# nicoloalbergoni/DeepLabV3Plus-Augmented-SuperResolution

Measured on AMD Instinct MI355X. Metric: augmented-copies/sec (fwd+realign+SR-iter) @512x512, higher is better.
Workload: dtype f32 (pointwise GEMMs: operands split into f16 hi+lo, hi*hi+hi*lo+lo*hi on f16 MFMA, f32 accumulate)

## Files before the change

### deeplabv3plus-augmented-superresolution_amd/csrc/dwconv.hip

```cpp
#include "asr_common.h"

typedef float f32x4 __attribute__((ext_vector_type(4)));

namespace {

struct DwArgs {
    const float* x;
    const float* w;
    const float* bias;
    float* y;
    int batch, h_in, w_in, c, h_out, w_out;
    int stride, rate, pad_top, pad_left;
    int pre_relu, post_relu;
    int ldx, ldy;
};

__device__ __forceinline__ f32x4 relu4(f32x4 v) {
    v.x = fmaxf(v.x, 0.f); v.y = fmaxf(v.y, 0.f); v.z = fmaxf(v.z, 0.f); v.w = fmaxf(v.w, 0.f);
    return v;
}
__device__ __forceinline__ f32x4 post_act4(f32x4 v, int mode) {
    if (mode) v = relu4(v);
    if (mode == 2) { v.x = fminf(v.x, 6.f); v.y = fminf(v.y, 6.f); v.z = fminf(v.z, 6.f); v.w = fminf(v.w, 6.f); }
    return v;
}

constexpr int SCOLS = 16;

template <int R, int S, int SROWS>
__global__ __launch_bounds__(256) void dw_stream_kernel(DwArgs p, int tiles_x) {
    constexpr int WIN = 2 * R + 1;
    const int tid = threadIdx.x;
    const int c4 = tid & 15, col = tid >> 4;
    const int tx = blockIdx.x % tiles_x, cbk = blockIdx.x / tiles_x;
    const int ch = (cbk * 16 + c4) * 4;
    const int ox = tx * SCOLS + col;
    const int oy0 = blockIdx.y * SROWS;
    const int b = blockIdx.z;
    if (ch >= p.c || ox >= p.w_out) return;
    const float* xin = p.x + (long long)b * p.h_in * p.w_in * p.ldx + ch;
    float* yout = p.y + (long long)b * p.h_out * p.w_out * p.ldy + ch;
    f32x4 wk[9];
#pragma unroll
    for (int t = 0; t < 9; ++t) wk[t] = *reinterpret_cast<const f32x4*>(p.w + (long long)t * p.c + ch);
    const f32x4 bv = *reinterpret_cast<const f32x4*>(p.bias + ch);
    const int ixl = ox * S - p.pad_left, ixc = ixl + R, ixr = ixl + 2 * R;
    const bool vl = ixl >= 0 && ixl < p.w_in, vc = ixc >= 0 && ixc < p.w_in, vr = ixr >= 0 && ixr < p.w_in;
    const f32x4 zero = {0.f, 0.f, 0.f, 0.f};

    auto load_row = [&](int iy, f32x4& l, f32x4& c, f32x4& r) {
        l = zero; c = zero; r = zero;
        if (iy >= 0 && iy < p.h_in) {
            const float* row = xin + (long long)iy * p.w_in * p.ldx;
            if (vl) l = *reinterpret_cast<const f32x4*>(row + (long long)ixl * p.ldx);
            if (vc) c = *reinterpret_cast<const f32x4*>(row + (long long)ixc * p.ldx);
            if (vr) r = *reinterpret_cast<const f32x4*>(row + (long long)ixr * p.ldx);
        }
    };
    auto act = [&](const f32x4& v) { return p.pre_relu ? relu4(v) : v; };

    f32x4 win[WIN][3], nxt[S][3];
    const int base0 = oy0 * S - p.pad_top;
#pragma unroll
    for (int k = 0; k < WIN - S; ++k) {
        load_row(base0 + k, win[S + k][0], win[S + k][1], win[S + k][2]);
        win[S + k][0] = act(win[S + k][0]); win[S + k][1] = act(win[S + k][1]); win[S + k][2] = act(win[S + k][2]);
    }
#pragma unroll
    for (int j = 0; j < S; ++j) load_row(base0 + WIN - S + j, nxt[j][0], nxt[j][1], nxt[j][2]);
    const int rows = min(SROWS, p.h_out - oy0);
    for (int r = 0; r < rows; ++r) {
#pragma unroll
        for (int k = 0; k < WIN - S; ++k) { win[k][0] = win[k + S][0]; win[k][1] = win[k + S][1]; win[k][2] = win[k + S][2]; }
#pragma unroll
        for (int j = 0; j < S; ++j) { win[WIN - S + j][0] = act(nxt[j][0]); win[WIN - S + j][1] = act(nxt[j][1]); win[WIN - S + j][2] = act(nxt[j][2]); }
        if (r + 1 < rows) {
#pragma unroll
            for (int j = 0; j < S; ++j) load_row(base0 + r * S + WIN + j, nxt[j][0], nxt[j][1], nxt[j][2]);
        }
        f32x4 acc = bv;
#pragma unroll
        for (int ky = 0; ky < 3; ++ky)
#pragma unroll
            for (int kx = 0; kx < 3; ++kx) acc += win[ky * R][kx] * wk[ky * 3 + kx];
        acc = post_act4(acc, p.post_relu);
        *reinterpret_cast<f32x4*>(yout + ((long long)(oy0 + r) * p.w_out + ox) * p.ldy) = acc;
    }
}

typedef _Float16 f16x4 __attribute__((ext_vector_type(4)));

#ifndef ASR_DIAG_DW
#define ASR_DIAG_DW 0
#endif
#ifndef ASR_DW_PACKED_SPLIT
#define ASR_DW_PACKED_SPLIT 1
#endif
typedef unsigned int dw_u32x2 __attribute__((ext_vector_type(2)));
__device__ __forceinline__ void dw_split4(const f32x4& acc, dw_u32x2& h2, dw_u32x2& l2) {
#if ASR_DW_PACKED_SPLIT
    unsigned int h01, h23, l01, l23;
    asr_split4_f16_saturating_mode(acc[0], acc[1], acc[2], acc[3], h01, h23, l01, l23);
    h2 = dw_u32x2{h01, h23};
    l2 = dw_u32x2{l01, l23};
#else
    f16x4 hi, lo;
#pragma unroll
    for (int e = 0; e < 4; ++e) {
        _Float16 h, l;
        asr_split_f16(acc[e], h, l);
        hi[e] = h;
        lo[e] = l;
    }
    h2 = __builtin_bit_cast(dw_u32x2, hi);
    l2 = __builtin_bit_cast(dw_u32x2, lo);
#endif
}

#ifndef ASR_DW_NT
#define ASR_DW_NT 1
#endif
constexpr bool kNtStores = ASR_DW_NT != 0;
#ifndef ASR_DW_SMALL_MAX
#define ASR_DW_SMALL_MAX 64
#endif
template <int R, int S, int SROWS, int PF, bool SPLIT, int ACT>
__global__ __launch_bounds__(256) ASR_PK_F32 void dw_stream_full_kernel(DwArgs p, int tiles_x) {
    constexpr int WIN = 2 * R + 1;
    static_assert(SROWS % PF == 0, "strip length must be a multiple of the prefetch depth");
#if ASR_DW_PACKED_SPLIT
    if (SPLIT) asr_enable_f16_saturation();
#endif
    const int tid = threadIdx.x;
    const int c4 = tid & 15, col = tid >> 4;
    const int tx = blockIdx.x % tiles_x, cbk = blockIdx.x / tiles_x;
    const int ch = (cbk * 16 + c4) * 4;
    const int ox = tx * SCOLS + col;
    const int oy0 = blockIdx.y * SROWS;
    const int b = blockIdx.z;
    _Float16* ysplit = nullptr;
    long long split_row_stride = 0;
    if (SPLIT) {
        ysplit = reinterpret_cast<_Float16*>(p.y) + (((long long)b * p.h_out * p.w_out + ox) * p.ldy + (ch >> 5)) * 64 + (ch & 31);
        split_row_stride = (long long)p.w_out * p.ldy * 64;
        if (ox < p.w_out && ch >= p.c && ch < p.ldy * 32) {
            const f16x4 z = {(_Float16)0.f, (_Float16)0.f, (_Float16)0.f, (_Float16)0.f};
            for (int r = 0; r < SROWS; ++r) {
                _Float16* o = ysplit + (long long)(oy0 + r) * split_row_stride;
                *reinterpret_cast<f16x4*>(o) = z;
                *reinterpret_cast<f16x4*>(o + 32) = z;
            }
        }
    }
    if (ch >= p.c || ox >= p.w_out) return;
    const float* xin = p.x + (long long)b * p.h_in * p.w_in * p.ldx + ch;
    float* yout = p.y + ((long long)b * p.h_out * p.w_out + ox) * p.ldy + ch;
    const int ixl = ox * S - p.pad_left, ixc = ixl + R, ixr = ixl + 2 * R;
    const bool vl = ixl >= 0 && ixl < p.w_in, vc = ixc >= 0 && ixc < p.w_in, vr = ixr >= 0 && ixr < p.w_in;
    const f32x4 zero = {0.f, 0.f, 0.f, 0.f};
    f32x4 wk[9];
#pragma unroll
    for (int t = 0; t < 9; ++t) {
        const bool col_ok = (t % 3 == 0) ? vl : ((t % 3 == 1) ? vc : vr);
        const f32x4 wv = *reinterpret_cast<const f32x4*>(p.w + (long long)t * p.c + ch);
        wk[t] = col_ok ? wv : zero;
    }
    const f32x4 bv = *reinterpret_cast<const f32x4*>(p.bias + ch);
    const long long ofl = (long long)min(max(ixl, 0), p.w_in - 1) * p.ldx, ofc = (long long)min(max(ixc, 0), p.w_in - 1) * p.ldx,
                    ofr = (long long)min(max(ixr, 0), p.w_in - 1) * p.ldx;
    const long long row_stride = (long long)p.w_in * p.ldx;
    const bool pre = ACT == 0 ? p.pre_relu != 0 : ACT == 1;

    auto issue = [&](int iy, f32x4 (&d)[3]) {
        const float* row = xin + (long long)min(max(iy, 0), p.h_in - 1) * row_stride;
#if ASR_DIAG_DW & 4
        d[1] = *reinterpret_cast<const f32x4*>(row + ofc);
        d[0] = d[1]; d[2] = d[1];
#else
        d[0] = *reinterpret_cast<const f32x4*>(row + ofl);
        d[1] = *reinterpret_cast<const f32x4*>(row + ofc);
        d[2] = *reinterpret_cast<const f32x4*>(row + ofr);
#endif
    };
    auto enter = [&](int iy, const f32x4 (&d)[3], f32x4 (&w)[3]) {
        const int vy = __builtin_amdgcn_readfirstlane((int)(iy >= 0 && iy < p.h_in));
#pragma unroll
        for (int k = 0; k < 3; ++k) w[k] = (ACT == 1) ? relu4(d[k]) : ((ACT == 2) ? d[k] : (pre ? relu4(d[k]) : d[k]));
        if (!vy) {
            asm volatile("" ::: "memory");
            w[0] = zero; w[1] = zero; w[2] = zero;
        }
    };

    f32x4 win[WIN][3], q[PF][S][3];
    const int base0 = oy0 * S - p.pad_top;
#pragma unroll
    for (int k = 0; k < WIN - S; ++k) {
        f32x4 d[3];
        issue(base0 + k, d);
        enter(base0 + k, d, win[S + k]);
    }
#pragma unroll
    for (int j = 0; j < PF; ++j)
#pragma unroll
        for (int t = 0; t < S; ++t) issue(base0 + WIN - S + j * S + t, q[j][t]);
#pragma unroll
    for (int r0 = 0; r0 < SROWS; r0 += PF) {
#pragma unroll
        for (int j = 0; j < PF; ++j) {
            const int r = r0 + j;
#pragma unroll
            for (int k = 0; k < WIN - S; ++k) { win[k][0] = win[k + S][0]; win[k][1] = win[k + S][1]; win[k][2] = win[k + S][2]; }
#pragma unroll
            for (int t = 0; t < S; ++t) enter(base0 + r * S + WIN - S + t, q[j][t], win[WIN - S + t]);
#pragma unroll
            for (int t = 0; t < S; ++t) issue(base0 + (r + PF) * S + WIN - S + t, q[j][t]);
            f32x4 acc = bv;
#if ASR_DIAG_DW & 1
            acc += win[R][1] * wk[4] + win[0][0] + win[2 * R][2];
#else
#pragma unroll
            for (int ky = 0; ky < 3; ++ky)
#pragma unroll
                for (int kx = 0; kx < 3; ++kx) acc += win[ky * R][kx] * wk[ky * 3 + kx];
#endif
            if (ACT == 2) acc = relu4(acc);
            else if (ACT == 0) acc = post_act4(acc, p.post_relu);
#if ASR_DIAG_DW & 2
            if (SPLIT) {
                _Float16* o = ysplit + (long long)(oy0 + r) * split_row_stride + ((c4 & 1) ? 32 - 4 : 0);
                __builtin_nontemporal_store(acc, reinterpret_cast<f32x4*>(o));
            } else
#endif
            if (SPLIT) {
                typedef dw_u32x2 u32x2;
                typedef unsigned int u32x4 __attribute__((ext_vector_type(4)));
                u32x2 h2, l2;
                dw_split4(acc, h2, l2);
                const bool even = (c4 & 1) == 0;
                const u32x2 give = even ? l2 : h2;
                u32x2 got;
                got.x = (unsigned int)__builtin_amdgcn_mov_dpp((int)give.x, 0xB1, 0xF, 0xF, true);
                got.y = (unsigned int)__builtin_amdgcn_mov_dpp((int)give.y, 0xB1, 0xF, 0xF, true);
                const u32x4 out = even ? u32x4{h2.x, h2.y, got.x, got.y} : u32x4{got.x, got.y, l2.x, l2.y};
                _Float16* o = ysplit + (long long)(oy0 + r) * split_row_stride + (even ? 0 : 32 - 4);
                if (kNtStores) __builtin_nontemporal_store(out, reinterpret_cast<u32x4*>(o)); else *reinterpret_cast<u32x4*>(o) = out;
            } else {
                if (kNtStores) __builtin_nontemporal_store(acc, reinterpret_cast<f32x4*>(yout + (long long)(oy0 + r) * p.w_out * p.ldy)); else *reinterpret_cast<f32x4*>(yout + (long long)(oy0 + r) * p.w_out * p.ldy) = acc;
            }
        }
    }
}


constexpr int ACB = 32;
constexpr int ATHREADS = 256;
constexpr int AMAXCOLS = 128;

struct AsppArgs {
    const float* x;
    const float* w;
    const float* bias;
    float* y[3];
    int batch, h, w_, c;
    int k[3];
    int g, nxg, gs;
    int ldx, ldy;
    int pre_relu, post_relu;
};

template <bool SPLIT>
__global__ __launch_bounds__(ATHREADS) void aspp_dw3_phase_kernel(AsppArgs p) {
#if ASR_DW_PACKED_SPLIT
    if (SPLIT) asr_enable_f16_saturation();
#endif
    extern __shared__ __attribute__((aligned(16))) float lds[];
    const int tid = threadIdx.x;
    const int c4 = tid & 7, slot = tid >> 3;
    const int cb = blockIdx.x * ACB;
    const int py = blockIdx.y / p.nxg, xg = blockIdx.y - py * p.nxg;
    const int b = blockIdx.z;
    const int g = p.g, gs = p.gs, x0 = xg * gs;
    const int rows = (p.h - py + g - 1) / g;
    const int qfull = (p.w_ - x0) / g, rem = (p.w_ - x0) - qfull * g;
    const int cols = (p.w_ > x0) ? qfull * gs + min(max(rem, 0), gs) : 0;
    const int lines = rows * cols;
    if (lines <= 0) return;
    int* xtab = reinterpret_cast<int*>(lds + (size_t)(lines + 1) * ACB);
    for (int j = tid; j < cols; j += ATHREADS) xtab[j] = (j / gs) * g + x0 + (j % gs);
    if (tid < 8) *reinterpret_cast<f32x4*>(lds + (size_t)lines * ACB + tid * 4) = f32x4{0.f, 0.f, 0.f, 0.f};
    const float* xin = p.x + (long long)b * p.h * p.w_ * p.ldx;
    const bool ch_ok = cb + c4 * 4 < p.c;
    {
        constexpr int UN = 8;
        const float* src = xin + (ch_ok ? cb + c4 * 4 : 0);
        const f32x4 zero = {0.f, 0.f, 0.f, 0.f};
        for (int base = slot; base < lines; base += 32 * UN) {
            f32x4 v[UN];
#pragma unroll
            for (int u = 0; u < UN; ++u) {
                const int l = min(base + u * 32, lines - 1);
                const int i = l / cols, j = l - i * cols;
                const int xx = (j / gs) * g + x0 + (j % gs);
                v[u] = *reinterpret_cast<const f32x4*>(src + ((long long)(py + i * g) * p.w_ + xx) * p.ldx);
            }
#pragma unroll
            for (int u = 0; u < UN; ++u) {
                const int l = base + u * 32;
                if (l < lines) *reinterpret_cast<f32x4*>(lds + (size_t)l * ACB + c4 * 4) = ch_ok ? (p.pre_relu ? relu4(v[u]) : v[u]) : zero;
            }
        }
    }
    __syncthreads();
    const int ch = cb + c4 * 4;
    if (ch >= p.c) return;
    const int zoff = lines * ACB + c4 * 4;
#pragma unroll 1
    for (int br = 0; br < 3; ++br) {
        const int k = p.k[br], kj = k * gs, kx_img = k * g;
        const float* wb = p.w + (long long)br * 9 * p.c + ch;
        f32x4 wk[9];
#pragma unroll
        for (int t = 0; t < 9; ++t) wk[t] = *reinterpret_cast<const f32x4*>(wb + (long long)t * p.c);
        const f32x4 bv = *reinterpret_cast<const f32x4*>(p.bias + (long long)br * p.c + ch);
        int i = slot / cols, j = slot - i * cols;
        for (int l = slot; l < lines; l += 32) {
            const int xx = xtab[j];
            const int center = (i * cols + j) * ACB + c4 * 4;
            const bool vyu = i - k >= 0, vyd = i + k < rows, vxl = xx - kx_img >= 0, vxr = xx + kx_img < p.w_;
            const int up = -k * cols * ACB, dn = k * cols * ACB, lf = -kj * ACB, rt = kj * ACB;
            f32x4 acc = bv;
            acc += *reinterpret_cast<const f32x4*>(lds + ((vyu && vxl) ? center + up + lf : zoff)) * wk[0];
            acc += *reinterpret_cast<const f32x4*>(lds + (vyu ? center + up : zoff)) * wk[1];
            acc += *reinterpret_cast<const f32x4*>(lds + ((vyu && vxr) ? center + up + rt : zoff)) * wk[2];
            acc += *reinterpret_cast<const f32x4*>(lds + (vxl ? center + lf : zoff)) * wk[3];
            acc += *reinterpret_cast<const f32x4*>(lds + center) * wk[4];
            acc += *reinterpret_cast<const f32x4*>(lds + (vxr ? center + rt : zoff)) * wk[5];
            acc += *reinterpret_cast<const f32x4*>(lds + ((vyd && vxl) ? center + dn + lf : zoff)) * wk[6];
            acc += *reinterpret_cast<const f32x4*>(lds + (vyd ? center + dn : zoff)) * wk[7];
            acc += *reinterpret_cast<const f32x4*>(lds + ((vyd && vxr) ? center + dn + rt : zoff)) * wk[8];
            acc = post_act4(acc, p.post_relu);
            const long long pix = (long long)b * p.h * p.w_ + (long long)(py + i * g) * p.w_ + xx;
            if (SPLIT) {
                typedef dw_u32x2 u32x2;
                typedef unsigned int u32x4 __attribute__((ext_vector_type(4)));
                u32x2 h2, l2;
                dw_split4(acc, h2, l2);
                const bool even = (c4 & 1) == 0;
                const u32x2 give = even ? l2 : h2;
                u32x2 got;
                got.x = (unsigned int)__builtin_amdgcn_mov_dpp((int)give.x, 0xB1, 0xF, 0xF, true);
                got.y = (unsigned int)__builtin_amdgcn_mov_dpp((int)give.y, 0xB1, 0xF, 0xF, true);
                const u32x4 out = even ? u32x4{h2.x, h2.y, got.x, got.y} : u32x4{got.x, got.y, l2.x, l2.y};
                _Float16* o = reinterpret_cast<_Float16*>(p.y[br]) + (pix * p.ldy + (cb >> 5)) * 64 + (even ? c4 * 4 : 32 + (c4 - 1) * 4);
                if (kNtStores) __builtin_nontemporal_store(out, reinterpret_cast<u32x4*>(o)); else *reinterpret_cast<u32x4*>(o) = out;
            } else {
                *reinterpret_cast<f32x4*>(p.y[br] + pix * p.ldy + ch) = acc;
            }
            j += 32;
            while (j >= cols) { j -= cols; ++i; }
        }
    }
}

__global__ __launch_bounds__(256) void dw_direct_kernel(DwArgs p) {
    const int c4n = p.c >> 2;
    const long long total = (long long)p.batch * p.h_out * p.w_out * c4n;
    for (long long o = (long long)blockIdx.x * 256 + threadIdx.x; o < total; o += (long long)gridDim.x * 256) {
        const int c4 = (int)(o % c4n);
        long long t = o / c4n;
        const int ox = (int)(t % p.w_out); t /= p.w_out;
        const int oy = (int)(t % p.h_out);
        const long long b = t / p.h_out;
        const int ch = c4 * 4;
        const float* xin = p.x + b * p.h_in * p.w_in * p.ldx;
        f32x4 acc = *reinterpret_cast<const f32x4*>(p.bias + ch);
#pragma unroll
        for (int ky = 0; ky < 3; ++ky) {
            const int iy = oy * p.stride - p.pad_top + ky * p.rate;
            if (iy < 0 || iy >= p.h_in) continue;
#pragma unroll
            for (int kx = 0; kx < 3; ++kx) {
                const int ix = ox * p.stride - p.pad_left + kx * p.rate;
                if (ix < 0 || ix >= p.w_in) continue;
                f32x4 v = *reinterpret_cast<const f32x4*>(xin + ((long long)iy * p.w_in + ix) * p.ldx + ch);
                if (p.pre_relu) v = relu4(v);
                acc += v * *reinterpret_cast<const f32x4*>(p.w + (long long)(ky * 3 + kx) * p.c + ch);
            }
        }
        acc = post_act4(acc, p.post_relu);
        *reinterpret_cast<f32x4*>(p.y + ((b * p.h_out + oy) * p.w_out + ox) * p.ldy + ch) = acc;
    }
}

template <int R, int S>
int launch_stream(const DwArgs& p, hipStream_t s, bool split = false) {
    const int tiles_x = (int)asr_cdiv(p.w_out, SCOLS), chunks = (int)asr_cdiv(p.c, 64);
    const int srows = p.h_out <= ASR_DW_SMALL_MAX ? 16 : 32;
    const dim3 grid(tiles_x * chunks, (unsigned)asr_cdiv(p.h_out, srows), p.batch);
    if (p.h_out % srows == 0) {
        const int act = (srows == 16) ? ((p.pre_relu == 1 && p.post_relu == 0) ? 1 : ((p.pre_relu == 0 && p.post_relu == 1) ? 2 : 0)) : 0;
#define ASR_DW_FULL(SR_, PF_, ACT_)                                                                                              \
    do {                                                                                                                         \
        if (split) hipLaunchKernelGGL((dw_stream_full_kernel<R, S, SR_, PF_, true, ACT_>), grid, dim3(256), 0, s, p, tiles_x);    \
        else hipLaunchKernelGGL((dw_stream_full_kernel<R, S, SR_, PF_, false, ACT_>), grid, dim3(256), 0, s, p, tiles_x);         \
    } while (0)
        if (srows == 32) ASR_DW_FULL(32, 1, 0);
        else if (act == 1) ASR_DW_FULL(16, 4, 1);
        else if (act == 2) ASR_DW_FULL(16, 4, 2);
        else ASR_DW_FULL(16, 4, 0);
#undef ASR_DW_FULL
        return ASR_OK;
    }
    ASR_UNSUPPORTED(split, "asr_dwconv3x3_nhwc_split_f16: needs h_out to be a multiple of the strip height (%d)", srows);
    if (srows == 16) hipLaunchKernelGGL((dw_stream_kernel<R, S, 16>), grid, dim3(256), 0, s, p, tiles_x);
    else hipLaunchKernelGGL((dw_stream_kernel<R, S, 32>), grid, dim3(256), 0, s, p, tiles_x);
    return ASR_OK;
}

}

extern "C" int asr_dwconv3x3_nhwc_f32(const float* x, const float* w, const float* bias, float* y, int batch, int h_in,
                                      int w_in, int c, int stride, int rate, int pad_top, int pad_left, int h_out,
                                      int w_out, int ldx, int ldy, int pre_relu, int post_relu, int mode,
                                      asr_stream_t stream) {
    ASR_REQUIRE(x && w && bias && y, "asr_dwconv3x3_nhwc_f32: null pointer");
    ASR_REQUIRE(batch > 0 && h_in > 0 && w_in > 0 && c > 0 && h_out > 0 && w_out > 0 && stride > 0 && rate > 0 &&
                    pad_top >= 0 && pad_left >= 0,
                "asr_dwconv3x3_nhwc_f32: bad geometry");
    ASR_REQUIRE(ldx >= c && ldy >= c, "asr_dwconv3x3_nhwc_f32: ldx/ldy < c");
    ASR_REQUIRE((long long)(h_out - 1) * stride - pad_top <= h_in - 1 && (long long)(w_out - 1) * stride - pad_left <= w_in - 1,
                "asr_dwconv3x3_nhwc_f32: output %dx%d does not fit input %dx%d (stride %d)", h_out, w_out, h_in, w_in, stride);
    ASR_UNSUPPORTED((c & 3) || (ldx & 3) || (ldy & 3), "asr_dwconv3x3_nhwc_f32: c, ldx, ldy must be multiples of 4");
    ASR_UNSUPPORTED((reinterpret_cast<uintptr_t>(x) | reinterpret_cast<uintptr_t>(y) | reinterpret_cast<uintptr_t>(w) |
// ... 128 lines not shown
```

### deeplabv3plus-augmented-superresolution_amd/csrc/gemm.hip

```cpp
#include "gemm_common.h"

namespace {

__device__ __forceinline__ void xcd_tile(int id, int count, int tiles_n, int& tile_m, int& tile_n) {
    const int q8 = count >> 3, r8 = count & 7, xcd = id & 7;
    const int lid = (xcd < r8 ? xcd * (q8 + 1) : r8 * (q8 + 1) + (xcd - r8) * q8) + (id >> 3);
    tile_m = lid / tiles_n;
    tile_n = lid % tiles_n;
}

template <int WM, int WN, int TM, int TN, bool CONV>
__global__ __launch_bounds__(256) void pw_gemm_kernel(PwArgs p) {
    constexpr int BM = WM * TM * 32, BN = WN * TN * 32;
    constexpr int A_F4 = BM / 32;
    constexpr int B_F4 = BN / 32;
    extern __shared__ __attribute__((aligned(16))) float smem[];
    float* const sA = smem;
    float* const sB = smem + BM * BK;

    int tile_m, tile_n;
    xcd_tile(blockIdx.x, gridDim.x, p.tiles_n, tile_m, tile_n);

    const int tid = threadIdx.x;
    const int lane = tid & 63, wave = tid >> 6;
// ... 301 lines not shown
            }
        }
        PHASE_MARK(2);
        if (kt + 1 < KT) {
            PHASE_WAIT_VM();
            PHASE_MARK(3);
            __syncthreads();
            PHASE_MARK(4);
            store_tile();
            PHASE_WAIT_LGKM();
            PHASE_MARK(5);
            __syncthreads();
            PHASE_MARK(6);
        }
    }
    __syncthreads();
    pw_epilogue<WM, WN, TM, TN>(p, acc, smem, tile_m, tile_n, wave, lane);
#ifdef ASR_GEMM_PHASE_PROFILE
    PHASE_MARK(7);
    if (tid == 0 && blockIdx.x < ASR_PHASE_BLOCKS)
        for (int i = 0; i < 8; ++i) g_phase_cycles[blockIdx.x * 16 + i] = ph[i];
#endif
}

namespace pre_ring {

constexpr int BM = 256, BN = 256, RT = 4, CT = 8;
constexpr int UNIT = 32 * 1024, RING = 5, B_PLANE = 4 * BN * 16;
constexpr int PIECES = 8;
static_assert(BM * 128 == UNIT && 2 * B_PLANE == UNIT, "unit size");

struct Loader {
    const PwArgs& p;
    char* const lds;
    const int wave, lane, first;
    const long long plane_bytes, kstep_b;
    unsigned off_a[PIECES], off_b[PIECES];
    const char* base_a;
    const char* base_b;

    __device__ __forceinline__ Loader(const PwArgs& p_, char* lds_, int wave_, int lane_)
        : p(p_), lds(lds_), wave(wave_), lane(lane_), first((wave_ - 8) * PIECES),
          plane_bytes((long long)p_.Kpad * p_.Npad * 2), kstep_b((long long)4 * p_.Npad * 16) {}

    __device__ __forceinline__ void setup(int tile_m, int tile_n) {
        const long long m0 = (long long)tile_m * BM;
        base_a = reinterpret_cast<const char*>(p.x) + m0 * p.ldx * 128;
        base_b = reinterpret_cast<const char*>(p.wp) + (long long)tile_n * BN * 16;
#pragma unroll
        for (int j = 0; j < PIECES; ++j) {
            const int pi = first + j;
            {
                const int q = pi * 64 + lane, row = q >> 3, slot = (q & 7) ^ ((row >> 1) & 7);
                long long r = row;
                if (m0 + r >= p.M) r = p.M - 1 - m0;
                off_a[j] = (unsigned)(r * p.ldx * 128 + slot * 16);
            }
            {
                const int qb = pi * 64 + lane, plane = qb >> 10, r = qb & 1023, oct = r >> 8, col = r & 255;
                off_b[j] = (unsigned)(plane * plane_bytes + ((long long)oct * p.Npad + col) * 16);
            }
        }
    }
    __device__ __forceinline__ void issue_a(int kt, int slot) {
        char* const dst = lds + slot * UNIT + first * 1024;
        const char* const src = base_a + (long long)kt * 128;
#pragma unroll
        for (int j = 0; j < PIECES; ++j) glds16_sbase(src, off_a[j], dst + j * 1024);
    }
    __device__ __forceinline__ void issue_b(int kt, int slot) {
        char* const dst = lds + slot * UNIT + first * 1024;
        const char* const src = base_b + kt * kstep_b;
#pragma unroll
        for (int j = 0; j < PIECES; ++j) glds16_sbase(src, off_b[j], dst + j * 1024);
    }
    __device__ __forceinline__ void issue_bias(int tile_n, int slot) {
        if (p.bias && wave == 8) {
            int col = tile_n * BN + lane * 4;
            if (col + 3 >= p.N) col = 0;
            glds16_sbase(p.bias, (unsigned)col * 4u, lds + slot * UNIT);
        }
    }
};

template <class Mark>
__device__ __forceinline__ void mfma_tile(const PwArgs& p, f32x4 (&acc)[RT][CT], const char* lds, int& slot, int KT, int tile_n,
                                          int lane, int wm, int wn, Mark&& mark) {
    const int ct_valid = min(CT, max(0, (p.N - (tile_n * BN + wn * (CT * 16)) + 15) >> 4));
#pragma unroll
    for (int i = 0; i < RT; ++i)
#pragma unroll
        for (int j = 0; j < CT; ++j)
#pragma unroll
            for (int e = 0; e < 4; ++e) acc[i][j][e] = 0.f;

    auto kloop = [&](auto CTV_) {
        constexpr int CTV = decltype(CTV_)::value;
        for (int kt = 0; kt < KT; ++kt) {
            const int off_a = slot * UNIT, off_b = (slot + 1 >= RING ? 0 : slot + 1) * UNIT;
            slot = slot + 2 >= RING ? slot + 2 - RING : slot + 2;
            int ln = lane;
            asm volatile("" : "+v"(ln));
            const int l16 = ln & 15, oct = ln >> 4;
            const int swz = (l16 >> 1) & 7;
            const int a_row = off_a + (wm * RT * 16 + l16) * 128;
            const int a_hi = a_row + ((oct ^ swz) << 4), a_lo = a_row + (((4 + oct) ^ swz) << 4);
            const int b_col = off_b + (oct * BN + wn * CT * 16 + l16) * 16;
            f16x8 ah[2], al[2], bh[2], bl[2];
            auto read_a = [&](int half, int i) {
                ah[i] = *reinterpret_cast<const f16x8*>(lds + a_hi + (2 * half + i) * 2048);
                al[i] = *reinterpret_cast<const f16x8*>(lds + a_lo + (2 * half + i) * 2048);
            };
            auto read_b = [&](int j, int buf) {
                bh[buf] = *reinterpret_cast<const f16x8*>(lds + b_col + j * 256);
                bl[buf] = *reinterpret_cast<const f16x8*>(lds + b_col + j * 256 + B_PLANE);
            };
            read_a(0, 0);
            read_a(0, 1);
            read_b(0, 0);
            auto group = [&](auto G) {
                constexpr int g = decltype(G)::value, half = g / CTV, j = g % CTV;
                constexpr bool last_of_half0 = g == CTV - 1;
                if (g + 1 < 2 * CTV) read_b((g + 1) % CTV, (g + 1) & 1);
#pragma unroll
                for (int i = 0; i < 2; ++i) {
                    f32x4& a4 = acc[2 * half + i][j];
                    a4 = __builtin_amdgcn_mfma_f32_16x16x32_f16(bh[g & 1], al[i], a4, 0, 0, 0);
                    a4 = __builtin_amdgcn_mfma_f32_16x16x32_f16(bl[g & 1], ah[i], a4, 0, 0, 0);
                    a4 = __builtin_amdgcn_mfma_f32_16x16x32_f16(bh[g & 1], ah[i], a4, 0, 0, 0);
                    if (last_of_half0) read_a(1, i);
                }
                if (g + 1 < 2 * CTV) __builtin_amdgcn_sched_group_barrier(0x100, 2, 0);
                __builtin_amdgcn_sched_group_barrier(0x008, 3, 0);
                if (last_of_half0) __builtin_amdgcn_sched_group_barrier(0x100, 2, 0);
                __builtin_amdgcn_sched_group_barrier(0x008, 3, 0);
                if (last_of_half0) __builtin_amdgcn_sched_group_barrier(0x100, 2, 0);
                __builtin_amdgcn_sched_barrier(0);
            };
            asr_static_for<2 * CTV>(group);
            asm volatile("s_waitcnt lgkmcnt(0)" ::: "memory");
            mark(2);
            __builtin_amdgcn_s_barrier();
            mark(6);
        }
    };
    if (ct_valid > 6) kloop(std::integral_constant<int, 8>{});
    else if (ct_valid > 4) kloop(std::integral_constant<int, 6>{});
    else if (ct_valid > 2) kloop(std::integral_constant<int, 4>{});
    else kloop(std::integral_constant<int, 2>{});
}

}

__global__ __launch_bounds__(768, 3) ASR_PK_F32 void pw_gemm_f16x3_pre_ring_kernel(PwArgs p) {
    using namespace pre_ring;
    extern __shared__ __attribute__((aligned(16))) float smem[];
    char* const lds = reinterpret_cast<char*>(smem);

    int tile_m, tile_n;
    xcd_tile(blockIdx.x, gridDim.x, p.tiles_n, tile_m, tile_n);
    const int tid = threadIdx.x, lane = tid & 63, wave = __builtin_amdgcn_readfirstlane(tid >> 6);
    const int KT = p.Kpad / BK;

    if (wave >= 8) {
        Loader ldr(p, lds, wave, lane);
        ldr.setup(tile_m, tile_n);
        ldr.issue_a(0, 0);
        ldr.issue_b(0, 1);
        if (KT > 1) {
            ldr.issue_a(1, 2);
            asm volatile("s_waitcnt vmcnt(8)" ::: "memory");
        } else {
            asm volatile("s_waitcnt vmcnt(0)" ::: "memory");
        }
        __builtin_amdgcn_s_barrier();
#ifdef ASR_GEMM_PHASE_PROFILE
        long long ph[8] = {0, 0, 0, 0, 0, 0, 0, 0};
        long long tprev = (long long)__builtin_readcyclecounter();
#endif
        int slot_b = 3, slot_a = 4;
        const bool ep_fast = pw_ep_fast(p);
        const bool res_dma = ep_fast && p.res != nullptr;
        auto issue_res = [&](int rt, int slot_h0, int slot_h1) {
#pragma unroll
            for (int j = 0; j < 16; ++j) {
                const int r = (wave - 8) * 16 + j;
                long long m = (long long)tile_m * BM + (r >> 4) * 64 + rt * 16 + (r & 15);
                if (m >= p.M) m = p.M - 1;
                int col = tile_n * BN + ((lane ^ (r & 15)) << 2);
                if (col + 3 >= p.N) col = 0;
                glds16_sbase(p.res + m * p.ldres, (unsigned)col * 4u, lds + ((r >> 5) ? slot_h1 : slot_h0) * UNIT + (r & 31) * 1024);
            }
        };
        for (int kt = 0; kt < KT; ++kt) {
            if (kt + 1 < KT) ldr.issue_b(kt + 1, slot_b);
            if (kt + 2 < KT) {
                ldr.issue_a(kt + 2, slot_a);
                PHASE_MARK(0);
                asm volatile("s_waitcnt vmcnt(8)" ::: "memory");
            } else {
                if (kt + 1 == KT && ep_fast) {
                    ldr.issue_bias(tile_n, slot_a);
                    if (res_dma) issue_res(0, slot_b - 1 < 0 ? RING - 1 : slot_b - 1, slot_b);
                }
                PHASE_MARK(0);
                asm volatile("s_waitcnt vmcnt(0)" ::: "memory");
            }
            PHASE_MARK(1);
            __builtin_amdgcn_s_barrier();
            PHASE_MARK(2);
            if (kt + 1 < KT) {
                slot_b = slot_b + 2 >= RING ? slot_b + 2 - RING : slot_b + 2;
                slot_a = slot_a + 2 >= RING ? slot_a + 2 - RING : slot_a + 2;
            }
        }
        if (res_dma) {
            const int b0h0 = slot_b - 1 < 0 ? RING - 1 : slot_b - 1, b0h1 = slot_b;
            const int b1h0 = (slot_b + 2) % RING, b1h1 = (slot_b + 3) % RING;
#pragma unroll 1
            for (int rt = 1; rt < 4; ++rt) {
                if (rt & 1) issue_res(rt, b1h0, b1h1); else issue_res(rt, b0h0, b0h1);
                asm volatile("s_waitcnt vmcnt(0)" ::: "memory");
                __builtin_amdgcn_s_barrier();
            }
        }
#ifdef ASR_GEMM_PHASE_PROFILE
        if (tid == 512 && blockIdx.x < ASR_PHASE_BLOCKS)
            for (int i = 0; i < 3; ++i) g_phase_cycles[blockIdx.x * 16 + 8 + i] = ph[i];
#endif
        return;
    }

    const int wm = wave & 3, wn = wave >> 2;
    f32x4 acc[RT][CT];
#ifdef ASR_GEMM_PHASE_PROFILE
    long long ph[8] = {0, 0, 0, 0, 0, 0, 0, 0};
    long long tprev = (long long)__builtin_readcyclecounter();
#endif
    __builtin_amdgcn_s_barrier();
    PHASE_MARK(0);
#ifdef ASR_GEMM_PHASE_PROFILE
    const long long loop_c0 = (long long)__builtin_readcyclecounter(), loop_r0 = (long long)__builtin_amdgcn_s_memrealtime();
#endif
    int slot = 0;
    mfma_tile(p, acc, lds, slot, KT, tile_n, lane, wm, wn, [&](int i) { PHASE_MARK(i); });
#ifdef ASR_GEMM_PHASE_PROFILE
    if (tid == 0 && blockIdx.x < ASR_PHASE_BLOCKS) {
        g_phase_cycles[blockIdx.x * 16 + 11] = (long long)__builtin_readcyclecounter() - loop_c0;
        g_phase_cycles[blockIdx.x * 16 + 12] = (long long)__builtin_amdgcn_s_memrealtime() - loop_r0;
    }
#endif
    pw_epilogue16_ring<RT, CT>(p, acc, lds, slot, UNIT, RING, (long long)tile_m * BM + wm * (RT * 16), tile_n * BN + wn * (CT * 16),
                              wm, wn);
#ifdef ASR_GEMM_PHASE_PROFILE
    asm volatile("s_waitcnt vmcnt(0)" ::: "memory");
    PHASE_MARK(7);
    if (tid == 0 && blockIdx.x < ASR_PHASE_BLOCKS)
        for (int i = 0; i < 8; ++i) g_phase_cycles[blockIdx.x * 16 + i] = ph[i];
#endif
}

__global__ __launch_bounds__(768, 3) ASR_PK_F32 void pw_gemm_f16x3_pre_ring_persist_kernel(PwArgs p, int ntiles) {
    using namespace pre_ring;
    extern __shared__ __attribute__((aligned(16))) float smem[];
    char* const lds = reinterpret_cast<char*>(smem);

    const int G = gridDim.x, wg = blockIdx.x;
    const int tid = threadIdx.x, lane = tid & 63, wave = __builtin_amdgcn_readfirstlane(tid >> 6);
    const int KT = p.Kpad / BK;
    int tile_m, tile_n;

    if (wave >= 8) {
        Loader ldr(p, lds, wave, lane);
        auto ring = [&](int v) { return v % RING; };
        const bool ep_fast = pw_ep_fast(p);
        int t = wg, s0 = 0;
        xcd_tile(t, ntiles, p.tiles_n, tile_m, tile_n);
        ldr.setup(tile_m, tile_n);
        ldr.issue_a(0, 0);
        ldr.issue_b(0, 1);
        asm volatile("s_waitcnt vmcnt(0)" ::: "memory");
        __builtin_amdgcn_s_barrier();
        for (; t < ntiles; t += G) {
            const bool has_next = t + G < ntiles;
            int slot_b = ring(s0 + 3), slot_a = ring(s0 + 4);
            for (int kt = 0; kt < KT; ++kt) {
                if (kt == 0) ldr.issue_a(1, ring(s0 + 2));
                if (kt + 1 < KT) ldr.issue_b(kt + 1, slot_b);
                if (kt + 2 < KT) {
                    ldr.issue_a(kt + 2, slot_a);
                    asm volatile("s_waitcnt vmcnt(8)" ::: "memory");
                } else {
                    if (kt + 1 == KT) {
                        if (ep_fast) ldr.issue_bias(tile_n, slot_a);
                        if (has_next) {
                            xcd_tile(t + G, ntiles, p.tiles_n, tile_m, tile_n);
                            ldr.setup(tile_m, tile_n);
                            ldr.issue_a(0, slot_b - 1 < 0 ? RING - 1 : slot_b - 1);
                            ldr.issue_b(0, slot_b);
                            asm volatile("s_waitcnt vmcnt(16)" ::: "memory");
                        } else {
                            asm volatile("s_waitcnt vmcnt(0)" ::: "memory");
                        }
                    } else {
                        asm volatile("s_waitcnt vmcnt(0)" ::: "memory");
                    }
                }
                __builtin_amdgcn_s_barrier();
                if (kt + 1 < KT) {
                    slot_b = slot_b + 2 >= RING ? slot_b + 2 - RING : slot_b + 2;
                    slot_a = slot_a + 2 >= RING ? slot_a + 2 - RING : slot_a + 2;
                }
            }
            asm volatile("s_waitcnt vmcnt(0)" ::: "memory");
            __builtin_amdgcn_s_barrier();
            s0 = ring(s0 + 2 * KT);
        }
        return;
    }

    const int wm = wave & 3, wn = wave >> 2;
    __builtin_amdgcn_s_barrier();
    int slot = 0;
    for (int t = wg; t < ntiles; t += G) {
        xcd_tile(t, ntiles, p.tiles_n, tile_m, tile_n);
        f32x4 acc[RT][CT];
        mfma_tile(p, acc, lds, slot, KT, tile_n, lane, wm, wn, [](int) {});
        pw_epilogue16_ring<RT, CT>(p, acc, lds, slot, UNIT, RING, (long long)tile_m * BM + wm * (RT * 16), tile_n * BN + wn * (CT * 16),
                                  wm, wn);
        asm volatile("s_waitcnt lgkmcnt(0)" ::: "memory");
        __builtin_amdgcn_s_barrier();
    }
}

__global__ __launch_bounds__(256) void pack_weights_f16x3_kernel(const float* __restrict__ w, _Float16* __restrict__ wp, int K,
                                                                 int N, int Kpad, int Npad) {
    const long long total = (long long)Kpad * Npad;
    for (long long o = (long long)blockIdx.x * 256 + threadIdx.x; o < total; o += (long long)gridDim.x * 256) {
        const int kr = (int)(o & 7);
        const long long t = o >> 3;
        const int n = (int)(t % Npad);
        const int k = (int)(t / Npad) * 8 + kr;
        const float v = (k < K && n < N) ? w[(long long)k * N + n] : 0.f;
        const _Float16 h = (_Float16)v;
        wp[o] = h;
        wp[total + o] = (_Float16)(v - (float)h);
    }
}

__global__ __launch_bounds__(256) void pack_weights_kernel(const float* __restrict__ w, float* __restrict__ wp, int K, int N,
                                                           int Kpad, int Npad) {
    const long long total = (long long)Kpad * Npad;
    for (long long o = (long long)blockIdx.x * 256 + threadIdx.x; o < total; o += (long long)gridDim.x * 256) {
        const int kr = (int)(o & 3);
        const long long t = o >> 2;
        const int n = (int)(t % Npad);
        const int k = (int)(t / Npad) * 4 + kr;
        wp[o] = (k < K && n < N) ? w[(long long)k * N + n] : 0.f;
    }
}

template <int WM, int WN, int TM, int TN, bool CONV>
int launch(const PwArgs& a, hipStream_t s) {
    constexpr int BM = WM * TM * 32, BN = WN * TN * 32;
    PwArgs p = a;
    p.tiles_n = (int)asr_cdiv(p.N, BN);
    const long long tiles_m = asr_cdiv(p.M, BM);
    const long long nwg = tiles_m * p.tiles_n;
    if (nwg > 0x7fffffffLL) {
        asr_set_error("asr_pwconv_mfma_f32: grid too large (%lld workgroups)", nwg);
        return ASR_ERR_INVALID_ARG;
    }
    const size_t lds = sizeof(float) * (BM * BK + BK * BN);
    auto kern = pw_gemm_kernel<WM, WN, TM, TN, CONV>;
    static AsrDeviceOnce once;
    ASR_HIP_CHECK(asr_allow_dynamic_lds(once, reinterpret_cast<const void*>(kern), (int)lds));
    hipLaunchKernelGGL(kern, dim3((unsigned)nwg), dim3(256), lds, s, p);
    ASR_LAUNCH_CHECK();
// ... 240 lines not shown
```

### deeplabv3plus-augmented-superresolution_amd/csrc/gemm_common.h

```cpp
#pragma once
#include "asr_common.h"
#include <utility>

typedef float f32x16 __attribute__((ext_vector_type(16)));
typedef float f32x4 __attribute__((ext_vector_type(4)));
typedef _Float16 f16x8 __attribute__((ext_vector_type(8)));

namespace {

constexpr int BK = 32;

struct PwArgs {
    const float* x;
    const float* wp;
    const float* bias;
    const float* res;
    float* y;
    long long M;
    int K, N, Npad, Kpad;
    int ldx, ldy, ldres;
    int relu;
    int tiles_n;
    int taps;
    int cin;
// ... 108 lines not shown
#pragma unroll
                for (int r = 0; r < 4; ++r) {
                    float v = acc[2 * i + h2][ct][r] + bv[ct];
                    if (p.relu) v = fmaxf(v, 0.f);
                    if (p.relu == 2) v = fminf(v, 6.f);
                    stage[(h2 * 16 + 4 * q4 + r) * WCOLS + ct * 16 + l16] = v;
                }
        if (res_vec && !kRequestFirst) {
            __builtin_amdgcn_sched_barrier(0);
#pragma unroll
            for (int q = 0; q < RES_DEPTH; ++q) request(q);
        }
#pragma unroll
        for (int q = 0; q < NQ; ++q) {
            const int r = q * RPI + r_in;
            const long long m = m_base + r;
            f32x4 v = *reinterpret_cast<const f32x4*>(stage + r * WCOLS + c4 * 4);
            f32x4 rq = {0.f, 0.f, 0.f, 0.f};
            if (res_vec) {
                rq = rv[q % RES_DEPTH];
                if (q + RES_DEPTH < NQ) request(q + RES_DEPTH);
            }
            if (m < p.M && n < p.N) {
                if (vec_ok) {
                    if (p.res) v += rq;
                    *reinterpret_cast<f32x4*>(p.y + m * p.ldy + n) = v;
                } else {
#pragma unroll
                    for (int t = 0; t < 4; ++t)
                        if (n + t < p.N) {
                            float o = v[t];
                            if (p.res) o += p.res[m * p.ldres + n + t];
                            p.y[m * p.ldy + n + t] = o;
                        }
                }
            }
        }
    }
}


__device__ __forceinline__ bool pw_ep_fast(const PwArgs& p) {
    return ((p.N & 3) == 0) && ((p.ldy & 3) == 0) && ((reinterpret_cast<uintptr_t>(p.y) & 15) == 0) &&
           ((reinterpret_cast<uintptr_t>(p.bias) & 15) == 0) &&
           (!p.res || (((p.ldres & 3) == 0) && ((reinterpret_cast<uintptr_t>(p.res) & 15) == 0)));
}

template <int RT, int CT>
__device__ __forceinline__ void pw_epilogue16_ring(const PwArgs& p, f32x4 (&acc)[RT][CT], const char* lds, int f, int unit, int ring,
                                                   long long m_wave, int n_wave, int wm, int wn) {
    int lane;
    {
        int z = 0;
        asm volatile("" : "+v"(z));
        lane = (int)__builtin_amdgcn_mbcnt_hi(~0u, __builtin_amdgcn_mbcnt_lo(~0u, (unsigned)z));
    }
    const int l16 = lane & 15, q4 = lane >> 4;
    const bool fast = pw_ep_fast(p);
    const bool res_dma = fast && p.res != nullptr;
    const bool rows_ok = m_wave + RT * 16 <= p.M;
    auto slot_of = [&](int k) { const int v = f + k; return v >= ring ? v - ring : v; };
    const int n0 = n_wave + 4 * q4;
    if (fast && rows_ok) {
        const char* const bias_lds = lds + slot_of(2) * unit + (wn * (CT * 16) + 4 * q4) * 4;
        const unsigned yoff = ((unsigned)l16 * (unsigned)p.ldy + (unsigned)n0) * 4u;
        const int relu = p.relu;
        const bool has_bias = p.bias != nullptr;
#pragma unroll
        for (int rt = 0; rt < RT; ++rt) {
            char* const yrow = reinterpret_cast<char*>(p.y + (m_wave + rt * 16) * p.ldy);
            const int r = wm * 16 + l16;
            const char* const res_lds = lds + slot_of((rt & 1) * 3 + (r >> 5)) * unit + (r & 31) * 1024;
            const int s0 = wn * (CT * 4) + q4;
#pragma unroll
            for (int ct = 0; ct < CT; ++ct) {
                if (n0 + ct * 16 < p.N) {
                    f32x4 v = acc[rt][ct];
                    if (has_bias) v += *reinterpret_cast<const f32x4*>(bias_lds + ct * 64);
                    if (relu) {
#pragma unroll
                        for (int t = 0; t < 4; ++t) v[t] = fmaxf(v[t], 0.f);
                    }
                    if (relu == 2) {
#pragma unroll
                        for (int t = 0; t < 4; ++t) v[t] = fminf(v[t], 6.f);
                    }
                    if (res_dma) v += *reinterpret_cast<const f32x4*>(res_lds + (((s0 + ct * 4) ^ l16) << 4));
                    *reinterpret_cast<f32x4*>(yrow + (yoff + ct * 64)) = v;
                }
            }
            if (res_dma && rt + 1 < RT) {
                asm volatile("s_waitcnt lgkmcnt(0)" ::: "memory");
                __builtin_amdgcn_s_barrier();
            }
        }
        return;
    }
    if (res_dma) {
#pragma unroll 1
        for (int rt = 0; rt + 1 < RT; ++rt) __builtin_amdgcn_s_barrier();
    }
#pragma unroll
    for (int ct = 0; ct < CT; ++ct) {
        const int n = n0 + ct * 16;
#pragma unroll
        for (int rt = 0; rt < RT; ++rt) {
            const long long m = m_wave + rt * 16 + l16;
            if (m >= p.M) continue;
#pragma unroll
            for (int t = 0; t < 4; ++t)
                if (n + t < p.N) {
                    float o = acc[rt][ct][t] + (p.bias ? p.bias[n + t] : 0.f);
                    if (p.relu) o = fmaxf(o, 0.f);
                    if (p.relu == 2) o = fminf(o, 6.f);
                    if (p.res) o += p.res[m * p.ldres + n + t];
                    p.y[m * p.ldy + n + t] = o;
                }
        }
    }
}

#ifdef ASR_GEMM_PHASE_PROFILE
#define ASR_PHASE_BLOCKS 8192
__device__ long long g_phase_cycles[ASR_PHASE_BLOCKS * 16];
#define PHASE_MARK(i)                                              \
    do {                                                           \
        const long long now_ = (long long)__builtin_readcyclecounter(); \
        ph[i] += now_ - tprev;                                     \
        tprev = now_;                                              \
    } while (0)
#define PHASE_WAIT_VM() asm volatile("s_waitcnt vmcnt(0)" ::: "memory")
#define PHASE_WAIT_LGKM() asm volatile("s_waitcnt lgkmcnt(0)" ::: "memory")
#else
#define PHASE_MARK(i)
#define PHASE_WAIT_VM()
#define PHASE_WAIT_LGKM()
#endif

typedef __attribute__((address_space(3))) void* asr_lds_ptr;
typedef const __attribute__((address_space(1))) void* asr_gbl_ptr;

__device__ __forceinline__ void glds16(const void* g, void* lds_wave_base) {
    __builtin_amdgcn_global_load_lds((asr_gbl_ptr)g, (asr_lds_ptr)lds_wave_base, 16, 0, 0);
}

__device__ __forceinline__ void glds16_sbase(const void* uniform_base, unsigned lane_byte_offset, void* lds_wave_base) {
    const unsigned m0v = (unsigned)(unsigned long long)(asr_lds_ptr)lds_wave_base;
    asm volatile("s_mov_b32 m0, %2\n\ts_nop 0\n\tglobal_load_lds_dwordx4 %0, %1"
                 :
                 : "v"(lane_byte_offset), "s"(uniform_base), "s"(m0v)
                 : "memory", "m0");
}

template <typename F, int... I>
__device__ __forceinline__ void asr_static_for_impl(F& f, std::integer_sequence<int, I...>) {
    (f(std::integral_constant<int, I>{}), ...);
}
template <int N, typename F>
__device__ __forceinline__ void asr_static_for(F& f) {
    asr_static_for_impl(f, std::make_integer_sequence<int, N>{});
}

inline int round_up(int v, int m) { return (v + m - 1) / m * m; }

}
```

Baseline: 2184.

## Prefetch residual tile into cache during GEMM tail; reverse depthwise block walk order

In the ring GEMM's residual-DMA path, producer waves issue dummy global loads that touch the residual tile rows during the last k-iterations. This warms the L2/MALL before the epilogue's residual DMA, with the vmcnt wait raised by one to account for the extra load. Separately, the depthwise and ASPP kernels walk grid y/z in descending order, presumably to reuse data left in cache by the preceding kernel. The extra loads add memory traffic and instruction overhead, and the reversed order could hurt locality if the previous kernel's access pattern differs.

```diff
diff --git a/deeplabv3plus-augmented-superresolution_amd/csrc/dwconv.hip b/deeplabv3plus-augmented-superresolution_amd/csrc/dwconv.hip
--- a/deeplabv3plus-augmented-superresolution_amd/csrc/dwconv.hip
+++ b/deeplabv3plus-augmented-superresolution_amd/csrc/dwconv.hip
@@ -27,6 +27,12 @@
 
 constexpr int SCOLS = 16;
 
+#ifndef ASR_DW_DESCEND
+#define ASR_DW_DESCEND 1
+#endif
+__device__ __forceinline__ int dw_walk_y() { return ASR_DW_DESCEND ? (int)(gridDim.y - 1 - blockIdx.y) : (int)blockIdx.y; }
+__device__ __forceinline__ int dw_walk_z() { return ASR_DW_DESCEND ? (int)(gridDim.z - 1 - blockIdx.z) : (int)blockIdx.z; }
+
 template <int R, int S, int SROWS>
 __global__ __launch_bounds__(256) void dw_stream_kernel(DwArgs p, int tiles_x) {
     constexpr int WIN = 2 * R + 1;
@@ -35,8 +41,8 @@
     const int tx = blockIdx.x % tiles_x, cbk = blockIdx.x / tiles_x;
     const int ch = (cbk * 16 + c4) * 4;
     const int ox = tx * SCOLS + col;
-    const int oy0 = blockIdx.y * SROWS;
-    const int b = blockIdx.z;
+    const int oy0 = dw_walk_y() * SROWS;
+    const int b = dw_walk_z();
     if (ch >= p.c || ox >= p.w_out) return;
     const float* xin = p.x + (long long)b * p.h_in * p.w_in * p.ldx + ch;
     float* yout = p.y + (long long)b * p.h_out * p.w_out * p.ldy + ch;
@@ -136,8 +142,8 @@
     const int tx = blockIdx.x % tiles_x, cbk = blockIdx.x / tiles_x;
     const int ch = (cbk * 16 + c4) * 4;
     const int ox = tx * SCOLS + col;
-    const int oy0 = blockIdx.y * SROWS;
-    const int b = blockIdx.z;
+    const int oy0 = dw_walk_y() * SROWS;
+    const int b = dw_walk_z();
     _Float16* ysplit = nullptr;
     long long split_row_stride = 0;
     if (SPLIT) {
@@ -278,8 +284,9 @@
     const int tid = threadIdx.x;
     const int c4 = tid & 7, slot = tid >> 3;
     const int cb = blockIdx.x * ACB;
-    const int py = blockIdx.y / p.nxg, xg = blockIdx.y - py * p.nxg;
-    const int b = blockIdx.z;
+    const int by = dw_walk_y();
+    const int py = by / p.nxg, xg = by - py * p.nxg;
+    const int b = dw_walk_z();
     const int g = p.g, gs = p.gs, x0 = xg * gs;
     const int rows = (p.h - py + g - 1) / g;
     const int qfull = (p.w_ - x0) / g, rem = (p.w_ - x0) - qfull * g;
diff --git a/deeplabv3plus-augmented-superresolution_amd/csrc/gemm.hip b/deeplabv3plus-augmented-superresolution_amd/csrc/gemm.hip
--- a/deeplabv3plus-augmented-superresolution_amd/csrc/gemm.hip
+++ b/deeplabv3plus-augmented-superresolution_amd/csrc/gemm.hip
@@ -477,6 +477,9 @@
 
 }
 
+#ifndef ASR_GEMM_RES_WARM
+#define ASR_GEMM_RES_WARM 4
+#endif
 __global__ __launch_bounds__(768, 3) ASR_PK_F32 void pw_gemm_f16x3_pre_ring_kernel(PwArgs p) {
     using namespace pre_ring;
     extern __shared__ __attribute__((aligned(16))) float smem[];
@@ -517,12 +520,38 @@
                 glds16_sbase(p.res + m * p.ldres, (unsigned)col * 4u, lds + ((r >> 5) ? slot_h1 : slot_h0) * UNIT + (r & 31) * 1024);
             }
         };
+        constexpr int kResWarm = ASR_GEMM_RES_WARM, kResTouches = 8;
+        const bool res_warm = kResWarm > 0 && res_dma;
+        const int warm_kt0 = max(KT - 1 - kResWarm, 0);
+        const long long res_m0 = (long long)tile_m * BM;
+        const int res_rows = (int)min(p.M - res_m0, (long long)BM);
+        const int res_g_last = max(res_rows - 8, 0);
+        const float* const res_tile = p.res + res_m0 * p.ldres;
+        unsigned res_off = 0, res_sink = 0;
+        if (res_warm) {
+            const int lrow = min(lane >> 3, res_rows - 1);
+            int col = tile_n * BN + (lane & 7) * 32;
+            if (col + 3 >= p.N) col = 0;
+            res_off = ((unsigned)lrow * (unsigned)p.ldres + (unsigned)col) * 4u;
+        }
+        auto touch_res = [&](int ti) {
+            const int rt = (1 + (ti >> 1)) & 3;
+            const int g0 = min((wave - 8) * 64 + rt * 16 + (ti & 1) * 8, res_g_last);
+            gtouch_sbase(res_tile + (long long)g0 * p.ldres, res_off, res_sink);
+        };
         for (int kt = 0; kt < KT; ++kt) {
             if (kt + 1 < KT) ldr.issue_b(kt + 1, slot_b);
             if (kt + 2 < KT) {
                 ldr.issue_a(kt + 2, slot_a);
-                PHASE_MARK(0);
-                asm volatile("s_waitcnt vmcnt(8)" ::: "memory");
+                const int ti = kt - warm_kt0;
+                if (res_warm && ti >= 0 && ti < kResTouches) {
+                    touch_res(ti);
+                    PHASE_MARK(0);
+                    asm volatile("s_waitcnt vmcnt(9)" ::: "memory");
+                } else {
+                    PHASE_MARK(0);
+                    asm volatile("s_waitcnt vmcnt(8)" ::: "memory");
+                }
             } else {
                 if (kt + 1 == KT && ep_fast) {
                     ldr.issue_bias(tile_n, slot_a);
@@ -549,6 +578,7 @@
                 __builtin_amdgcn_s_barrier();
             }
         }
+        asm volatile("" : : "v"(res_sink));
 #ifdef ASR_GEMM_PHASE_PROFILE
         if (tid == 512 && blockIdx.x < ASR_PHASE_BLOCKS)
             for (int i = 0; i < 3; ++i) g_phase_cycles[blockIdx.x * 16 + 8 + i] = ph[i];
diff --git a/deeplabv3plus-augmented-superresolution_amd/csrc/gemm_common.h b/deeplabv3plus-augmented-superresolution_amd/csrc/gemm_common.h
--- a/deeplabv3plus-augmented-superresolution_amd/csrc/gemm_common.h
+++ b/deeplabv3plus-augmented-superresolution_amd/csrc/gemm_common.h
@@ -284,6 +284,10 @@
                  : "memory", "m0");
 }
 
+__device__ __forceinline__ void gtouch_sbase(const void* uniform_base, unsigned lane_byte_offset, unsigned& sink) {
+    asm volatile("s_nop 4\n\tglobal_load_dword %0, %1, %2" : "+v"(sink) : "v"(lane_byte_offset), "s"(uniform_base) : "memory");
+}
+
 template <typename F, int... I>
 __device__ __forceinline__ void asr_static_for_impl(F& f, std::integer_sequence<int, I...>) {
     (f(std::integral_constant<int, I>{}), ...);
```

After: 2193, median of 5. No clear change (+0.4%).
